# martingleich/RayTracingInAWeekend

Hardware: AMD Instinct MI355X
Metric: Msamples/sec at 1920x1080x512spp; achieved HBM GB/s vs peak (higher is better)
Workload: dtype f32

## Files before the change

include/rtw.h:

```cpp
#ifndef RTW_H
#define RTW_H

#include <stddef.h>
#include <stdint.h>

#ifdef __cplusplus
extern "C" {
#endif

#define RTW_API __attribute__((visibility("default")))
#define RTW_ABI_VERSION 2

#define RTW_OK 0
#define RTW_ERR_INVALID_ARGUMENT 1
#define RTW_ERR_NO_DEVICE 2
#define RTW_ERR_HIP 3
#define RTW_ERR_OUT_OF_MEMORY 4
#define RTW_ERR_UNSUPPORTED 5
#define RTW_ERR_IO 6
#define RTW_ERR_PARSE 7

#define RTW_GEOM_SPHERE 0
#define RTW_GEOM_RECT 1
#define RTW_GEOM_BOX 2
// ... 175 lines not shown
                                float* out_rgb, rtw_progress_fn cb, void* user);

RTW_API int rtw_render_devices(const rtw_world* world, const rtw_render_params* params, const int* devices,
                               int n_devices, float* out_rgb);
typedef struct rtw_multi rtw_multi;
RTW_API int rtw_multi_create(const rtw_world* world, const int* devices, int n_devices, rtw_multi** out);
RTW_API int rtw_multi_render(rtw_multi* m, const rtw_render_params* params, float* d_image);
RTW_API int rtw_multi_release(rtw_multi* m);
RTW_API int rtw_multi_peer_copies(const rtw_multi* m, uint64_t* copies);

RTW_API int rtw_world_upload(const rtw_world* world, int device, rtw_gpu_world** out);
RTW_API int rtw_world_release(rtw_gpu_world* gw);
RTW_API int rtw_world_tuning(rtw_gpu_world* gw, int* trace_min);
RTW_API int rtw_world_kernel(rtw_gpu_world* gw, int* lds_mode, int* leaf_kinds, int* tex_kinds, int* tree);
RTW_API int rtw_world_kernel_name(rtw_gpu_world* gw, char* buf, int cap);
RTW_API int rtw_world_last_frame(rtw_gpu_world* gw, int* launches, int* whole_pixel, int* trace_min);
RTW_API int rtw_world_last_frame_lists(rtw_gpu_world* gw, int* listed, int* empty, int* walked, double* mean_len);
RTW_API int rtw_world_primary_lists(rtw_gpu_world* gw, int32_t* n_tiles, int32_t* cap, double* build_ms,
                                    int32_t* count, int32_t* list);
RTW_API int rtw_primary_lists_host(const rtw_world* world, const rtw_render_params* params, int32_t cap,
                                   int32_t* count, int32_t* list);
RTW_API int rtw_render_device(rtw_gpu_world* gw, const rtw_render_params* params, float* d_out,
                              void* stream);
typedef struct rtw_accum rtw_accum;
#define RTW_ACCUM_MOMENTS 1u
#define RTW_ACCUM_ADAPTIVE 2u
#define RTW_ACCUM_FINITE 4u
typedef struct rtw_accum_info {
    uint32_t version;
    uint32_t flags;
// ... 187 lines not shown
```

raytracinginaweekend_amd/_native.py:

```python
from __future__ import annotations

import ctypes as C
import os

_HERE = os.path.dirname(os.path.abspath(__file__))
LIB_PATH = os.environ.get("RTW_LIBRARY") or os.path.join(_HERE, "librtw.so")

RTW_OK = 0
RTW_ERR_INVALID_ARGUMENT = 1
RTW_ERR_NO_DEVICE = 2
RTW_ERR_HIP = 3
RTW_ERR_OUT_OF_MEMORY = 4
RTW_ERR_UNSUPPORTED = 5
RTW_ERR_IO = 6
RTW_ERR_PARSE = 7

GEOM_SPHERE, GEOM_RECT, GEOM_BOX, GEOM_TRIANGLE = 0, 1, 2, 3
PLANE_XY, PLANE_XZ, PLANE_YZ = 0, 1, 2
MAT_LAMBERT, MAT_METAL, MAT_DIELECTRIC, MAT_DIFFUSE_LIGHT, MAT_ISOTROPIC = 0, 1, 2, 3, 4
TEX_SOLID, TEX_CHECKER, TEX_MARBLE, TEX_IMAGE = 0, 1, 2, 3
BG_SKY, BG_SOLID = 0, 1
MODE_DEFAULT, MODE_NORMALS = 0, 1
LEAF_VOLUME, LEAF_TRANSFORM, LEAF_ANIMATION = 1, 2, 4
LAYOUT_IMAGE, LAYOUT_TILES = 0, 1
# ... 254 lines not shown

ABI_VERSION = 2
_lib = None

_P = C.c_void_p
_SIGS = {
    "rtw_version": (C.c_int, []),
    "rtw_last_error": (C.c_char_p, []),
    "rtw_device_count": (C.c_int, [C.POINTER(C.c_int)]),
    "rtw_render": (C.c_int, [C.POINTER(World), C.POINTER(RenderParams), C.c_int, C.POINTER(C.c_float)]),
    "rtw_world_upload": (C.c_int, [C.POINTER(World), C.c_int, C.POINTER(_P)]),
    "rtw_world_release": (C.c_int, [_P]),
    "rtw_world_tuning": (C.c_int, [_P, C.POINTER(C.c_int)]),
    "rtw_world_kernel": (C.c_int, [_P] + [C.POINTER(C.c_int)] * 4),
    "rtw_world_kernel_name": (C.c_int, [_P, C.c_char_p, C.c_int]),
    "rtw_world_last_frame": (C.c_int, [_P] + [C.POINTER(C.c_int)] * 3),
    "rtw_world_last_frame_lists": (C.c_int, [_P] + [C.POINTER(C.c_int)] * 3 + [C.POINTER(C.c_double)]),
    "rtw_world_primary_lists": (C.c_int, [_P, C.POINTER(C.c_int32), C.POINTER(C.c_int32), C.POINTER(C.c_double),
                                          C.POINTER(C.c_int32), C.POINTER(C.c_int32)]),
    "rtw_primary_lists_host": (C.c_int, [C.POINTER(World), C.POINTER(RenderParams), C.c_int32, C.POINTER(C.c_int32),
                                         C.POINTER(C.c_int32)]),
    "rtw_render_device": (C.c_int, [_P, C.POINTER(RenderParams), _P, _P]),
    "rtw_render_devices": (C.c_int, [C.POINTER(World), C.POINTER(RenderParams), C.POINTER(C.c_int), C.c_int,
                                     C.POINTER(C.c_float)]),
    "rtw_multi_create": (C.c_int, [C.POINTER(World), C.POINTER(C.c_int), C.c_int, C.POINTER(_P)]),
    "rtw_multi_render": (C.c_int, [_P, C.POINTER(RenderParams), _P]),
    "rtw_multi_release": (C.c_int, [_P]),
    "rtw_multi_peer_copies": (C.c_int, [_P, C.POINTER(C.c_uint64)]),
    "rtw_world_fingerprint": (C.c_int, [C.POINTER(World), C.POINTER(C.c_uint64)]),
    "rtw_accum_create": (C.c_int, [_P, C.POINTER(RenderParams), C.c_uint32, C.POINTER(_P)]),
# ... 149 lines not shown
```

raytracinginaweekend_amd/csrc/rtw_device.hip:

```cpp
#include <hip/hip_runtime.h>

#include <algorithm>
#include <cmath>
#include <limits>
#include <cstdio>
#include <cstdlib>
#include <cstring>
#include <ctime>
#include <string>
#include <type_traits>
#include <vector>

#include "../../include/rtw_scalar.h"
#include "../../include/rtw_cull.h"
#include "../../include/rtw_beam.h"
#include "../../include/rtw_adapt.h"
#include "../../include/rtw_finite.h"
#include "../../include/rtw_parts.h"
#include "rtw_common.h"

#ifndef RTW_BLOCK
#define RTW_BLOCK 1024
#endif
#ifndef RTW_MIN_WAVES_PER_SIMD
// ... 143 lines not shown
    int32_t whole_pixel;
    const uint32_t* tile_perm;
    uint32_t* slot_cost;
    uint32_t chunks;
    uint64_t big_from;
    FastDiv fd_total, fd_rank, fd_tile, fd_tiles_x, fd_tile_w;
    FastDiv fd_spread, fd_epoch, fd_half;
    int32_t sh_xf, sh_sph, sh_bx, sh_rect;
    int32_t sphere_count, box_count;
    int32_t mb_off, mb_cap;
    int32_t tri_prefix, tri_stride;
    int32_t tri_prefix_mat, tri_prefix_w;
    const int32_t* pl_count;
    const int32_t* pl_list;
    int32_t pl_cap, pl_shade_min;
};

struct V3 {
    float x, y, z;
};
__host__ __device__ __forceinline__ V3 v3(float x, float y, float z) { return V3{x, y, z}; }
__host__ __device__ __forceinline__ V3 add(V3 a, V3 b) { return v3(a.x + b.x, a.y + b.y, a.z + b.z); }
__host__ __device__ __forceinline__ V3 sub(V3 a, V3 b) { return v3(a.x - b.x, a.y - b.y, a.z - b.z); }
__device__ __forceinline__ V3 neg(V3 a) { return v3(-a.x, -a.y, -a.z); }
__host__ __device__ __forceinline__ V3 mul(V3 a, float s) { return v3(a.x * s, a.y * s, a.z * s); }
__device__ __forceinline__ V3 divs(V3 a, float s) { return v3(a.x / s, a.y / s, a.z / s); }
__device__ __forceinline__ V3 conv(V3 a, V3 b) { return v3(a.x * b.x, a.y * b.y, a.z * b.z); }
__host__ __device__ __forceinline__ float dot(V3 a, V3 b) { return a.x * b.x + a.y * b.y + a.z * b.z; }
__host__ __device__ __forceinline__ V3 cross(V3 a, V3 b) {
    return v3(a.y * b.z - a.z * b.y, a.z * b.x - a.x * b.z, a.x * b.y - a.y * b.x);
// ... 946 lines not shown
        float d0, d1;
        d_unit_disc(&rng, d0, d1);
        off = mul(add(mul(ld3(c.unit_right), d0), mul(ld3(c.unit_up), d1)), c.lens_radius);
    }
    float start;
    if (c.time0 == c.time1) start = c.time0;
    else start = d_gen_range_f32(c.time0, c.time1, &rng);
    Ray r;
    r.time = start + (c.shutter_pace[0] * px + c.shutter_pace[1] * py);
    r.o = add(ld3(c.position), off);
    r.d = unit_x(sub(sub(add(ld3(c.upper_left_corner), mul(ld3(c.scaled_right), px)), mul(ld3(c.scaled_up), py)), off));
    return r;
}

#ifdef RTW_PHASE_TIMING
__device__ unsigned long long rtw_phase_cycles[8];
__device__ __forceinline__ unsigned long long* pt_slot() {
    __shared__ unsigned long long s[(RTW_BLOCK / 64) * 10];
    return s + (threadIdx.x >> 6) * 10;
}
#define RTW_PT_DECL do { unsigned long long* s_ = pt_slot(); if ((threadIdx.x & 63) == 0) { for (int k_ = 0; k_ < 8; ++k_) s_[k_] = 0; s_[8] = clock64(); s_[9] = 0; } } while (0);
#define RTW_PT(k) do { if ((int)(threadIdx.x & 63) == __ffsll((long long)__ballot(1)) - 1) { unsigned long long* s_ = pt_slot(); const unsigned long long now_ = clock64(); s_[s_[9]] += now_ - s_[8]; s_[8] = now_; s_[9] = (k); } } while (0)
#define RTW_PT_FLUSH do { RTW_PT(0); if ((threadIdx.x & 63) == 0) for (int k_ = 0; k_ < 8; ++k_) atomicAdd(&rtw_phase_cycles[k_], pt_slot()[k_]); } while (0)
#else
#define RTW_PT_DECL
#define RTW_PT(k) do { } while (0)
#define RTW_PT_FLUSH do { } while (0)
#endif

struct Path {
    Ray ray;
    V3 att, acc;
    int32_t depth;
    rtw_xoro rng;
};
struct ShadeOut {
    Path p;
    V3 color;
    int32_t done;
    uint32_t texels;
};
// ... 121 lines not shown
                }
        }
    } else {
        color = add(acc, conv(att, background(w.wc->bg, pdot)));
        done = true;
    }
    ShadeOut o;
    o.p = P;
    o.color = color;
    o.done = done ? 1 : 0;
    o.texels = STATS ? st.c[ST_TEXEL] : 0u;
    return o;
}

__device__ unsigned long long rtw_drain_counts[3];

#ifdef RTW_WAVE_TIMING
__device__ unsigned long long rtw_wave_times[3 * 8192];
__device__ unsigned long long rtw_wave_dry[8192];
__device__ unsigned long long rtw_wave_extra[8 * 8192];
#endif

enum { PH_PIXEL = 0, PH_TRACE = 1, PH_SHADE = 2, PH_REF = 3, PH_DONE = 4 };
enum { TM_REF = 0, TM_SAH = 1, TM_FALLBACK = 2 };
#define RTW_TF_SAH 16
#define RTW_TF_TIE 32


struct Trav {
    Ray ray;
// ... 348 lines not shown
        if (__builtin_amdgcn_readfirstlane((int)ok)) {
            j = (int)(si & 0xFFu);
            return uu;
        }
    }
}

__device__ __forceinline__ void sah_take(Trav& T, float t, int leaf) {
    const bool same = T.found >= 0 && t == __int_as_float(__float_as_int(T.te) - 1);
    const bool tie = same && T.found != leaf;
    T.fast = same ? (tie ? (T.fast | RTW_TF_TIE) : T.fast) : (T.fast & ~RTW_TF_TIE);
    T.te = same ? T.te : __int_as_float(__float_as_int(t) + 1);
    T.found = same ? T.found : leaf;
}

template <bool STATS, int LDS, int LK, int TX, bool GEN, bool WP, bool PL = false>
__device__ __forceinline__ void render_body(const KArgs& A) {
    static_assert(!PL || (LDS == 1 && LK == LK_SPHERES && !GEN), "leaf lists: plain-sphere worlds, LDS mode 1");
    constexpr bool LDS_SCENE = LDS >= 1;
    const DWorld& w = A.w;
    constexpr bool SAHK = LK <= LK_WRAPPED;
    const bool sah = SAHK && A.sah != 0;
    if (LDS_SCENE) {
        const float4* ga = sah ? w.sah_a : w.node_a;
        const float4* gb = sah ? w.sah_b : w.node_b;
        for (int i = threadIdx.x; i < A.node_count; i += RTW_BLOCK) {
            smem[i] = ga[i];
            smem[A.node_count + i] = gb[i];
        }
        const int32_t n_rec = A.leaf_count - A.tri_prefix;
        for (int i = threadIdx.x; i < n_rec; i += RTW_BLOCK) smem[2 * A.node_count + i] = w.leaf_fast[A.tri_prefix + i];
        const bool km_rec = sah && LK == LK_SPHERES;
        const int32_t km_f4 = km_rec ? 0 : (A.node_count + 1) / 2;
// ... 80 lines not shown
        fresh = true;
        if (PL) cam = true;
        RTW_PT(back);
    };

    int32_t trace_min = A.trace_min;
    bool tuned = true;
    if (A.tune) {
        const int ch = __hip_atomic_load(&A.tune->chosen, __ATOMIC_RELAXED, __HIP_MEMORY_SCOPE_AGENT);
        if (ch > 0) trace_min = ch;
        else tuned = A.tune_items == 0;
    }
    uint64_t w_next = 0, w_end = 0;
    uint32_t wq = (blockIdx.x * (RTW_BLOCK / 64) + (threadIdx.x >> 6)) % RTW_QUEUES;
    uint32_t qfail = 0;
    unsigned long long pf_b = 0;
    uint64_t pf_size = 0;
    int pf_lane = 0;
    auto prefetch = [&](int leader) {
        const uint64_t rest = A.q_cap > w_end ? A.q_cap - w_end : 0;
        const uint64_t cap = w_end * RTW_QUEUES >= A.big_from ? RTW_WAVE_BATCH_BIG : RTW_WAVE_BATCH;
        pf_size = max((uint64_t)1, min(cap, (uint64_t)fdiv((uint32_t)rest, A.fd_spread)));
        if (lane == leader) pf_b = atomicAdd(A.queue + wq * RTW_QSTRIDE, (unsigned long long)pf_size);
        pf_lane = leader;
    };
    RTW_PT_DECL
#ifdef RTW_WAVE_TIMING
    uint32_t wx_busy = 0, wx_n = 0, wx_sum = 0, wx_max = 0, wx_coop = 0, wx_ref = 0;
    uint64_t wx_tref = 0, wx_tsah = 0, wx_tcoop = 0;
    bool wx_dry = false;
#endif
    static_assert(!(GEN && WP), "GEN kernels take whole-pixel items at run time");
    const bool WPX = GEN ? A.whole_pixel != 0 : WP;
    constexpr bool SHARE_K = !STATS && LDS_SCENE && LK == LK_TRIS;
    int32_t mb_v = SHARE_K ? A.mb_off : -1;
    asm volatile("" : "+v"(mb_v));
    auto share_on = [&]() { return SHARE_K && __builtin_amdgcn_readfirstlane(mb_v) >= 0; };
    auto mailbox = [&]() { return reinterpret_cast<uint32_t*>(smem + __builtin_amdgcn_readfirstlane(mb_v)); };
    for (;;) {
        if (__ballot(T.phase != PH_DONE) == 0) break;
        RTW_PT(1);
        for (;;) {
            const unsigned long long m = __ballot(T.phase == PH_PIXEL);
            if (m == 0) break;
            if (qfail >= RTW_QUEUES) {
#ifdef RTW_WAVE_TIMING
                {
                    const uint32_t wv_ = (blockIdx.x * RTW_BLOCK + threadIdx.x) / 64;
                    if (wv_ < 8192) atomicMin(&rtw_wave_dry[wv_], (unsigned long long)wall_clock64());
                }
#endif
#ifdef RTW_WAVE_TIMING
                if (!wx_dry) wx_busy = (uint32_t)__popcll(__ballot(T.phase != PH_PIXEL));
                wx_dry = true;
#endif
                if (T.phase == PH_PIXEL) T.phase = PH_DONE;
// ... 13 lines not shown
                empty = base >= A.q_cap;
                w_next = empty ? A.q_cap : base;
                w_end = empty ? A.q_cap : min(base + size, A.q_cap);
                if (!tuned && wq == 0 && !empty) {
                    const uint64_t H = A.fd_half.d;
                    const uint64_t g0 = base * RTW_QUEUES, g1 = (base + size) * RTW_QUEUES;
                    const uint64_t j = fdiv((uint32_t)min(g0 + H - 1, (uint64_t)0xFFFFFFFFu), A.fd_half);
                    if (lane == leader && j >= 1 && j <= RTW_TUNE_STAMPS && j * H < g1)
                        __hip_atomic_store(&A.tune->tb[j - 1], wall_clock64(), __ATOMIC_RELAXED,
                                           __HIP_MEMORY_SCOPE_AGENT);
                }
            }
            const uint64_t left = min(need, w_end - w_next);
            const uint64_t first = w_next;
            w_next += left;
            if (!tuned) {
                const uint64_t e = fdiv((uint32_t)min(w_next * RTW_QUEUES, (uint64_t)0xFFFFFFFFu), A.fd_epoch);
                if (e == 0) {
                    trace_min = A.trace_min;
                } else if (e <= RTW_TUNE_EPOCHS) {
                    const int i = (int)e - 1;
                    trace_min = kTuneCand[i < RTW_TUNE_NCAND ? i : RTW_TUNE_EPOCHS - 1 - i];
                } else {
                    const unsigned long long* tbp = A.tune->tb;
                    auto stamp = [&](int k) {
                        return __hip_atomic_load(&tbp[k], __ATOMIC_RELAXED, __HIP_MEMORY_SCOPE_AGENT);
                    };
                    bool ok = stamp(0) != ~0ull && stamp(1) != ~0ull;
                    unsigned long long best_t = 0;
                    int best = A.trace_min;
// ... 66 lines not shown
                wq = (wq + 1) % RTW_QUEUES;
                ++qfail;
                w_next = w_end = 0;
            } else if (took) {
                qfail = 0;
            }
        }

        RTW_PT(2);
        uint64_t c_trav = 0;
        if (STATS) {
            c_trav = clock64();
            if (lane == __ffsll((long long)__ballot(1)) - 1)
                atomicAdd(&A.stats[ST_COUNT + DB_REST_CYCLES], (unsigned long long)(c_trav - c_mark));
        }
        if (fresh) {
            fresh = false;
            const RayPre rp = ray_pre(T.ray, A.mk_world != 0);
            T.inv = rp.inv;
            T.fast = (rp.fast ? 8 : 0) | (T.ray.d.x > 0.0f ? 1 : 0) | (T.ray.d.y > 0.0f ? 2 : 0) | (T.ray.d.z > 0.0f ? 4 : 0);
            T.node = w.root;
            if (sah) {
                if (rp.fast) {
                    T.node = LK == LK_SPHERES ? w.sah_root_c2 : w.sah_root;
                    T.fast |= RTW_TF_SAH;
                } else {
                    T.phase = PH_REF;
                }
            }
            T.sp = 0;
            T.te = F32_INF;
            T.found = -1;
            if (STATS) st.c[ST_RAYS]++;
            if constexpr (PL) {
                if (cam && rp.fast && sah) {
                    const uint32_t tile = (uint32_t)A.part_index + fdiv(slot, A.fd_tile) * (uint32_t)A.part_count;
                    const int32_t n = A.pl_count[tile];
                    if (n >= 0) {
                        const int32_t* __restrict__ L = A.pl_list + (size_t)tile * (uint32_t)A.pl_cap;
                        const float4* fast = smem + A.fast_off;
                        for (int32_t j = 0; j < n; ++j) {
                            const int32_t leaf = L[j];
                            float t;
                            if (STATS) st.c[ST_T_SPHERE]++;
                            if (sphere_t(fast[leaf], T.ray, 0.001f, T.te, t)) sah_take(T, t, leaf);
                        }
                        T.phase = PH_SHADE;
                    }
                }
            }
        }

        RTW_PT(3);
        if (sah) {
            const bool dry_coop = !STATS && LK <= LK_PLAIN && qfail >= RTW_QUEUES && A.coop_max > 0;
#ifdef RTW_WAVE_TIMING
            uint64_t wx_t0 = wall_clock64();
#endif
            int32_t tmin = __builtin_amdgcn_readfirstlane(trace_min);
            if (PL && (int32_t)__popcll(__ballot(T.phase == PH_SHADE)) >= A.pl_shade_min) tmin = 65;
            T = traverse<STATS, LDS, LK, true, TM_SAH>(A.wdev, stabs, T, tmin, A.node_count,
                                                       A.leaf_count, A.rect_count, A.tri_prefix, A.tri_stride, stack_off,
                                                       STATS ? A.stats + ST_COUNT : nullptr, dry_coop ? A.coop_max : -1);
// ... 185 lines not shown
                }
                if (STATS) st.c[ST_SAMPLES]++;
                const int32_t bounces = A.max_depth - depth;
                if (!STATS && A.slot_cost && bounces > 3) {
                    if (WPX) pcost += (uint32_t)bounces;
                    else atomicAdd(&A.slot_cost[slot], (uint32_t)bounces);
                }
#ifdef RTW_WAVE_TIMING
                if (qfail >= RTW_QUEUES) {
                    ++wx_n;
                    wx_sum += (uint32_t)bounces;
                    wx_max = max(wx_max, (uint32_t)bounces);
                }
#endif
                ++sample;
                if (sample >= sample_end) {
                    T.phase = PH_PIXEL;
                    if (WPX) {
                        if (!STATS && A.slot_cost && pcost) atomicAdd(&A.slot_cost[slot], pcost);
                        const V3 px = divs(psum, (float)A.spp);
                        float* o = A.layout == RTW_LAYOUT_TILES ? A.out + 3 * (size_t)slot : A.out + 3 * (size_t)pix;
                        o[0] = px.x;
                        o[1] = px.y;
                        o[2] = px.z;
                    }
                } else {
                    start_sample(7);
                }
            } else {
                fresh = true;
                if (PL) cam = false;
// ... 22 lines not shown
            a.sgn = __float_as_int(q1.w);
            a.inv = v3(q2.x, q2.y, q2.z);
            const CHit h = coop_solve<LDS, LK>(w, a, A.node_count, A.leaf_count, A.rect_count, A.fast_off, A.tri_prefix,
                                               A.tri_stride, A.coop_ties == 2);
            if (lane == 0) {
                mb_answer(mb, q, u, h);
                __hip_atomic_fetch_add(&mb[34], 1u, __ATOMIC_RELAXED, __HIP_MEMORY_SCOPE_WORKGROUP);
            }
        }
        __syncthreads();
        if (threadIdx.x < 3) {
            const uint32_t c = __hip_atomic_load(&mb[33 + threadIdx.x], __ATOMIC_RELAXED, __HIP_MEMORY_SCOPE_WORKGROUP);
            if (c) atomicAdd(&rtw_drain_counts[threadIdx.x], (unsigned long long)c);
        }
    }
    RTW_PT_FLUSH;
#ifdef RTW_WAVE_TIMING
    {
        const uint32_t wv_ = (blockIdx.x * RTW_BLOCK + threadIdx.x) / 64;
        if (wv_ < 8192) {
            unsigned long long* x = rtw_wave_extra + 8 * wv_;
            if (wx_busy) atomicMax(&x[0], (unsigned long long)wx_busy);
            atomicAdd(&x[1], (unsigned long long)wx_n);
            atomicAdd(&x[2], (unsigned long long)wx_sum);
            (void)wx_max;
            if (lane == 0) {
                x[4] = wx_coop;
                x[5] = wx_ref;
                x[6] = wx_tref;
                x[7] = wx_tsah;
// ... 15 lines not shown
#endif
    render_body<STATS, LDS, LK, TX, GEN, WP>(A);
#ifdef RTW_WAVE_TIMING
    const uint32_t wv = (blockIdx.x * RTW_BLOCK + threadIdx.x) / 64;
    if ((threadIdx.x & 63) == 0 && wv < 8192) {
        rtw_wave_times[3 * wv] = t_start;
        rtw_wave_times[3 * wv + 1] = wall_clock64();
        rtw_wave_times[3 * wv + 2] = rtw_wave_dry[wv];
        rtw_wave_dry[wv] = ~0ull;
    }
#endif
}
template <bool STATS, int LDS, int LK, int TX, bool GEN = false, bool WP = false>
__global__ __launch_bounds__(RTW_BLOCK, RTW_MIN_WAVES_PER_SIMD) void render_kernel_pl(KArgs A) {
    render_body<STATS, LDS, LK, TX, GEN, WP, true>(A);
}

#define RTW_PL_GROUP 64
__global__ __launch_bounds__(RTW_PL_GROUP) void primary_lists_kernel(const rtw_camera* __restrict__ cam,
                                                                      const float4* __restrict__ fast, int32_t leaf_count,
                                                                      int32_t W, int32_t H, int32_t tw, int32_t th,
                                                                      int32_t tiles_x, int32_t n_tiles, int32_t cap,
                                                                      int32_t* __restrict__ count, int32_t* __restrict__ list) {
    const int32_t tile = (int32_t)blockIdx.x;
    if (tile >= n_tiles) return;
    const int lane = threadIdx.x;
    rtw_beam_tile t;
    rtw_beam_tile_setup(cam, W, H, tw, th, tile % tiles_x, tile / tiles_x, &t);
    int32_t n = 0;
    bool walk = !t.ok;
// ... 1138 lines not shown
    uint64_t order_key[10] = {};
    hipEvent_t done = nullptr;
    bool done_recorded = false;
    uint32_t order_tiles = 0;
    bool order_valid = false;
    int32_t last_kernel[6] = {-1, -1, -1, -1, -1, -1};
    int32_t last_frame[4] = {-1, -1, -1, 0};
    bool pl_scope = false;
    int32_t* pl_buf = nullptr;
    int32_t pl_key[5] = {0, 0, 0, 0, 0};
    int32_t pl_tiles = 0;
    int32_t pl_info[3] = {0, 0, 0};
    double pl_mean = 0.0;
    double pl_build_ms = 0.0;
    int32_t last_pl = 0;
    int32_t last_lists[3] = {0, 0, 0};
    double last_mean = 0.0;
    uint64_t fingerprint = 0;
    std::vector<struct rtw_accum*> accums;
    std::vector<struct rtw_aov*> aovs;
};

extern "C" RTW_API int rtw_debug_wave_times(unsigned long long* out24576) {
#ifdef RTW_WAVE_TIMING
    HIP_TRY(hipDeviceSynchronize());
    HIP_TRY(hipMemcpyFromSymbol(out24576, HIP_SYMBOL(rtw_wave_times), 3 * 8192 * sizeof(unsigned long long)));
    return RTW_OK;
#else
    (void)out24576;
    return rtw::fail(RTW_ERR_UNSUPPORTED, "built without RTW_WAVE_TIMING");
// ... 12 lines not shown
#endif
}

extern "C" RTW_API int rtw_debug_drain_counts(int device, unsigned long long* out3, int reset) {
    if (!out3) return rtw::fail(RTW_ERR_INVALID_ARGUMENT, "null argument");
    HIP_TRY(hipSetDevice(device));
    HIP_TRY(hipDeviceSynchronize());
    HIP_TRY(hipMemcpyFromSymbol(out3, HIP_SYMBOL(rtw_drain_counts), 3 * sizeof(unsigned long long)));
    if (reset) {
        unsigned long long z[3] = {};
        HIP_TRY(hipMemcpyToSymbol(HIP_SYMBOL(rtw_drain_counts), z, sizeof(z)));
    }
    return RTW_OK;
}

extern "C" RTW_API int rtw_debug_phase_cycles(unsigned long long* out8) {
#ifdef RTW_PHASE_TIMING
    HIP_TRY(hipDeviceSynchronize());
    HIP_TRY(hipMemcpyFromSymbol(out8, HIP_SYMBOL(rtw_phase_cycles), 8 * sizeof(unsigned long long)));
    unsigned long long z[8] = {};
    HIP_TRY(hipMemcpyToSymbol(HIP_SYMBOL(rtw_phase_cycles), z, sizeof(z)));
    return RTW_OK;
#else
    (void)out8;
    return rtw::fail(RTW_ERR_UNSUPPORTED, "built without RTW_PHASE_TIMING");
#endif
}

extern "C" RTW_API int rtw_device_count(int* count) {
    if (!count) return rtw::fail(RTW_ERR_INVALID_ARGUMENT, "null count");
    int n = 0;
    hipError_t e = hipGetDeviceCount(&n);
    if (e != hipSuccess) n = 0;
    *count = n;
    return RTW_OK;
}

extern "C" RTW_API int rtw_world_upload(const rtw_world* w, int device, rtw_gpu_world** out) {
    if (!out) return rtw::fail(RTW_ERR_INVALID_ARGUMENT, "null out");
// ... 384 lines not shown
}

extern "C" RTW_API int rtw_world_kernel(rtw_gpu_world* g, int* lds_mode, int* leaf_kinds, int* tex_kinds, int* tree) {
    if (!g || !lds_mode || !leaf_kinds || !tex_kinds || !tree) return rtw::fail(RTW_ERR_INVALID_ARGUMENT, "null argument");
    *lds_mode = g->last_kernel[0];
    *leaf_kinds = g->last_kernel[1];
    *tex_kinds = g->last_kernel[2];
    *tree = g->last_kernel[3];
    return RTW_OK;
}

extern "C" RTW_API int rtw_world_kernel_name(rtw_gpu_world* g, char* buf, int cap) {
    if (!g || !buf || cap < 1) return rtw::fail(RTW_ERR_INVALID_ARGUMENT, "null argument");
    char s[64] = "";
    if (g->last_kernel[0] >= 0)
        std::snprintf(s, sizeof(s), "render_kernel%s<false, %d, %d, %d, %s, %s>", g->last_pl ? "_pl" : "", g->last_kernel[0], g->last_kernel[1],
                      g->last_kernel[2], g->last_kernel[4] ? "true" : "false", g->last_kernel[5] ? "true" : "false");
    if ((int)std::strlen(s) >= cap) return rtw::fail(RTW_ERR_INVALID_ARGUMENT, "buffer too small");
    std::memcpy(buf, s, std::strlen(s) + 1);
    return RTW_OK;
}

extern "C" RTW_API int rtw_world_last_frame(rtw_gpu_world* g, int* launches, int* whole_pixel, int* trace_min) {
    if (!g || !launches || !whole_pixel || !trace_min) return rtw::fail(RTW_ERR_INVALID_ARGUMENT, "null argument");
    *launches = g->last_frame[0];
    *whole_pixel = g->last_frame[1];
    *trace_min = g->last_frame[2];
    if (g->last_frame[3]) {
        HIP_TRY(hipSetDevice(g->device));
        int v = 0;
        HIP_TRY(hipMemcpy(&v, &g->tune->chosen, sizeof(int), hipMemcpyDeviceToHost));
        if (v > 0) *trace_min = v;
// ... 45 lines not shown
                                      w->leaf_count, cap, list + (size_t)t * cap);
    return RTW_OK;
}

static void accum_orphan(struct rtw_accum* a);
static void aov_orphan(struct rtw_aov* a);

extern "C" RTW_API int rtw_world_release(rtw_gpu_world* g) {
    if (!g) return RTW_OK;
    (void)hipSetDevice(g->device);
    for (struct rtw_accum* a : g->accums) accum_orphan(a);
    for (struct rtw_aov* a : g->aovs) aov_orphan(a);
    if (g->arena) (void)hipFree(g->arena);
    if (g->queue) (void)hipFree(g->queue);
    if (g->colors) (void)hipFree(g->colors);
    if (g->tune) (void)hipFree(g->tune);
    if (g->slot_cost) (void)hipFree(g->slot_cost);
    if (g->tile_buf) (void)hipFree(g->tile_buf);
    if (g->sort_tmp) (void)hipFree(g->sort_tmp);
    if (g->running) (void)hipFree(g->running);
    if (g->pl_buf) (void)hipFree(g->pl_buf);
    if (g->done) (void)hipEventDestroy(g->done);
    delete g;
    return RTW_OK;
}

namespace {

int make_args(const rtw_gpu_world* g, const rtw_render_params* p, KArgs& A) {
    if (!g || !p) return rtw::fail(RTW_ERR_INVALID_ARGUMENT, "null argument");
// ... 42 lines not shown
    A.wdev = g->wdev;
    A.trace_min = 32;
    A.stats_tree = 0;
    if (const char* e = getenv("RTW_TRACE_MIN")) A.trace_min = atoi(e);
    A.seed_key = rtw_seed_key(p->seed);
    A.sx = 1.0f / (float)(p->width - 1);
    A.sy = 1.0f / (float)(p->height - 1);
    A.ux = rtw_uniform_new(0.0f, 1.0f / (float)(p->width - 1));
    A.uy = rtw_uniform_new(0.0f, 1.0f / (float)(p->height - 1));
    return RTW_OK;
}

enum LaunchKind { LK_RENDER, LK_STATS };
size_t env_size(const char* name, size_t dflt);
constexpr int RTW_ACC_NO_WP = -1;
int launch_render(rtw_gpu_world* g, KArgs& A, int kind, hipStream_t stream, bool acc_wp = false) {
    const bool stats = kind == LK_STATS;
    const bool ktree = stats && A.stats_tree == 1;
    int lk = g->leaf_kinds, tx = g->tex_kinds;
    if (const char* e = std::getenv("RTW_LEAF_KINDS")) lk = std::max(lk, std::min(4, std::atoi(e)));
    if (const char* e = std::getenv("RTW_TEX_KINDS")) tx = std::max(tx, std::min(1, std::atoi(e)));
    const bool sah = (!stats || ktree) && g->sah_nodes > 0 && g->mk_world && lk <= LK_WRAPPED &&
                     g->sah_folded == (lk == LK_SPHERES);
    A.sah = sah ? 1 : 0;
    A.coop_max = g->leaf_count <= RTW_COOP_LEAVES ? (int32_t)env_size("RTW_COOP_MAX", RTW_COOP_MAX) : 0;
    if (const char* e = std::getenv("RTW_COOP_MAX"))
        if (e[0] == '0') A.coop_max = 0;
    A.coop_ties = g->leaf_count <= RTW_COOP_LEAVES && g->w.leaf_key != nullptr ? 1 : 0;
    if (const char* e = std::getenv("RTW_COOP_TIES"))
        if (e[0] == '0') A.coop_ties = 0;
    if (const char* e = std::getenv("RTW_COOP_AUDIT"))
        if (e[0] == '1' && A.coop_ties) A.coop_ties = 2;
    const int blocks_per_cu = std::max(1, (4 * RTW_MIN_WAVES_PER_SIMD * 64) / RTW_BLOCK);
    size_t cap = std::min({(size_t)RTW_LDS_SCENE_MAX, (size_t)g->lds_max, (size_t)g->lds_cu / blocks_per_cu});
#ifdef RTW_PHASE_TIMING
    cap -= (RTW_BLOCK / 64) * 10 * sizeof(unsigned long long);
#endif
    const size_t stack_bytes = (size_t)g->depth * RTW_BLOCK * sizeof(int32_t);
    const size_t stack16_bytes = stack_bytes / 2;
    const char* lds_mode_env = std::getenv("RTW_LDS_MODE");
    A.node_count = sah ? g->sah_nodes : g->node_count;
    const int kernel_lk = stats && !sah ? (int)LK_ANY : lk;
    A.tri_prefix = kernel_lk == LK_TRIS ? g->tri_prefix : 0;
    A.tri_stride = kernel_lk == LK_TRIS ? std::max(1, g->tri_count) : RTW_TRI_SOA;
    const size_t tri_bytes = (size_t)4 * A.tri_stride * sizeof(float4);
    const size_t scene_bytes =
        (size_t)(2 * A.node_count + g->leaf_count - A.tri_prefix + (sah && lk == LK_SPHERES ? 0 : (A.node_count + 1) / 2) +
                 2 * g->rect_count) * sizeof(float4);
    A.fast_off = 2 * A.node_count - A.tri_prefix;
    if (A.fast_off < 0) return rtw::fail(RTW_ERR_UNSUPPORTED, "triangle prefix longer than the node records");
    int mode = 0;
// ... 75 lines not shown
#undef RTW_SSET
#define RTW_GSET(TX)                                                                                     \
    {{render_kernel<false, 1, LK_WRAPPED, TX, true>, render_kernel<false, 2, LK_WRAPPED, TX, true>}, \
     {render_kernel<false, 1, LK_ANY, TX, true>, render_kernel<false, 2, LK_ANY, TX, true>}}
    static const KFn fns_gen[2][2][2] = {RTW_GSET(TX_SOLID), RTW_GSET(TX_ANY)};
#undef RTW_GSET
    const bool gen = !stats && A.sh_xf >= 0;
    if (gen && tx != TX_SOLID && A.sh_tex0 >= 0)
        return rtw::fail(RTW_ERR_UNSUPPORTED, "GEN kernel with a texture table in LDS");
    if (gen && acc_wp) return RTW_ACC_NO_WP;
    const int wp = A.whole_pixel ? 1 : 0;
    KFn kf = stats ? (sah ? fns_stats_sah[lk][mode] : fns_stats[mode])
             : gen   ? fns_gen[tx][lk - LK_WRAPPED][mode - 1]
                     : fns[wp][tx][lk][mode];
    static const KFn fns_pl[2][2] = {
        {render_kernel_pl<false, 1, LK_SPHERES, TX_SOLID, false, false>, render_kernel_pl<false, 1, LK_SPHERES, TX_ANY, false, false>},
        {render_kernel_pl<false, 1, LK_SPHERES, TX_SOLID, false, true>, render_kernel_pl<false, 1, LK_SPHERES, TX_ANY, false, true>}};
    const bool pl = (!stats || ktree) && !gen && A.pl_count != nullptr && sah && lk == LK_SPHERES && mode == 1;
    if (pl) kf = stats ? render_kernel_pl<true, 1, LK_SPHERES, TX_ANY> : fns_pl[wp][tx];
    else A.pl_count = nullptr;
    if (!stats) {
        g->last_pl = pl ? 1 : 0;
        g->last_kernel[0] = mode;
        g->last_kernel[1] = lk;
        g->last_kernel[2] = tx;
        g->last_kernel[3] = sah ? 1 : 0;
        g->last_kernel[4] = gen ? 1 : 0;
        g->last_kernel[5] = gen ? 0 : wp;
    }
    const void* fn = (const void*)kf;
    HIP_TRY(hipFuncSetAttribute(fn, hipFuncAttributeMaxDynamicSharedMemorySize, (int)lds));
    int per_cu = 0;
    HIP_TRY(hipOccupancyMaxActiveBlocksPerMultiprocessor(&per_cu, fn, RTW_BLOCK, lds));
    if (per_cu < 1) return rtw::fail(RTW_ERR_UNSUPPORTED, "render kernel does not fit on a CU");
    const int64_t want = (int64_t)((A.items + RTW_BLOCK - 1) / RTW_BLOCK);
    const int64_t blocks = std::max<int64_t>(1, std::min<int64_t>(want, (int64_t)per_cu * g->cus));
    HIP_TRY(hipMemsetAsync(A.queue, 0, RTW_QUEUE_BLOCK * sizeof(unsigned long long), stream));
    A.tune_items = 0;
    if (A.tune && A.total > 0 && !A.tile_perm) {
        const uint64_t lanes = (uint64_t)blocks * RTW_BLOCK;
        const uint64_t E = (uint64_t)A.total * ((2 * lanes + A.total - 1) / A.total);
        if (A.items_big >= (uint64_t)(RTW_TUNE_EPOCHS + 2) * E) {
            A.tune_items = E;
            HIP_TRY(hipMemsetAsync(A.tune->tb, 0xFF, sizeof(A.tune->tb), stream));
        }
    }
    A.fd_spread = fastdiv_make((uint32_t)std::max<int64_t>(1, RTW_BATCH_SPREAD * blocks * (RTW_BLOCK / 64) / RTW_QUEUES));
    A.fd_epoch = fastdiv_make((uint32_t)std::max<uint64_t>(1, A.tune_items));
    A.fd_half = fastdiv_make((uint32_t)std::max<uint64_t>(1, A.tune_items / 2));
    hipLaunchKernelGGL(kf, dim3((unsigned)blocks), dim3(RTW_BLOCK), lds, stream, A);
    HIP_TRY(hipGetLastError());
// ... 1383 lines not shown
```

raytracinginaweekend_amd/rendering.py:

```python
from __future__ import annotations

import ctypes as C
import enum
from dataclasses import dataclass

import numpy as np

from . import _native as N
from ._native import check, lib
from .world import World


class RenderMode(enum.IntEnum):
    Default = N.MODE_DEFAULT
    Normals = N.MODE_NORMALS


@dataclass(frozen=True)
class Size2i:
    width: int
    height: int

    def count(self) -> int:
        return self.width * self.height
# ... 131 lines not shown
        v = C.c_int()
        check(lib().rtw_world_tuning(self._h, C.byref(v)))
        return v.value

    def kernel_variant(self) -> dict:
        m, lk, tx, tr = C.c_int(), C.c_int(), C.c_int(), C.c_int()
        check(lib().rtw_world_kernel(self._h, C.byref(m), C.byref(lk), C.byref(tx), C.byref(tr)))
        name = C.create_string_buffer(64)
        check(lib().rtw_world_kernel_name(self._h, name, 64))
        out = {"lds_mode": m.value, "leaf_kinds": lk.value, "tex_kinds": tx.value,
               "tree": ("reference", "sah")[tr.value] if tr.value >= 0 else None,
               "name": name.value.decode()}
        out.update(self._lists())
        return out

    def last_frame(self) -> dict:
        if not hasattr(lib(), "rtw_world_last_frame"):
            return {"launches": None, "whole_pixel": None, "trace_min": self.tuned_trace_min()}
        n, wp, tm = C.c_int(), C.c_int(), C.c_int()
        check(lib().rtw_world_last_frame(self._h, C.byref(n), C.byref(wp), C.byref(tm)))
        out = {"launches": n.value, "whole_pixel": bool(wp.value == 1), "trace_min": tm.value}
        out.update(self._lists())
        return out

    def _lists(self) -> dict:
        if not hasattr(lib(), "rtw_world_last_frame_lists"):
            return {}
        a, b, c, m = C.c_int(), C.c_int(), C.c_int(), C.c_double()
        check(lib().rtw_world_last_frame_lists(self._h, C.byref(a), C.byref(b), C.byref(c), C.byref(m)))
        return {"tiles_listed": a.value, "tiles_empty": b.value, "tiles_walked": c.value,
# ... 55 lines not shown
```

Measured before the change: 8771.

## Batch camera-ray generation per wave and park rays in a global buffer

```diff
diff --git a/include/rtw.h b/include/rtw.h
--- a/include/rtw.h
+++ b/include/rtw.h
@@ -213,6 +213,7 @@
 RTW_API int rtw_world_tuning(rtw_gpu_world* gw, int* trace_min);
 RTW_API int rtw_world_kernel(rtw_gpu_world* gw, int* lds_mode, int* leaf_kinds, int* tex_kinds, int* tree);
 RTW_API int rtw_world_kernel_name(rtw_gpu_world* gw, char* buf, int cap);
+RTW_API int rtw_debug_park_counts(int device, unsigned long long* out3, int reset);
 RTW_API int rtw_world_last_frame(rtw_gpu_world* gw, int* launches, int* whole_pixel, int* trace_min);
 RTW_API int rtw_world_last_frame_lists(rtw_gpu_world* gw, int* listed, int* empty, int* walked, double* mean_len);
 RTW_API int rtw_world_primary_lists(rtw_gpu_world* gw, int32_t* n_tiles, int32_t* cap, double* build_ms,
diff --git a/raytracinginaweekend_amd/_native.py b/raytracinginaweekend_amd/_native.py
--- a/raytracinginaweekend_amd/_native.py
+++ b/raytracinginaweekend_amd/_native.py
@@ -292,6 +292,7 @@
     "rtw_world_tuning": (C.c_int, [_P, C.POINTER(C.c_int)]),
     "rtw_world_kernel": (C.c_int, [_P] + [C.POINTER(C.c_int)] * 4),
     "rtw_world_kernel_name": (C.c_int, [_P, C.c_char_p, C.c_int]),
+    "rtw_debug_park_counts": (C.c_int, [C.c_int, C.POINTER(C.c_ulonglong), C.c_int]),
     "rtw_world_last_frame": (C.c_int, [_P] + [C.POINTER(C.c_int)] * 3),
     "rtw_world_last_frame_lists": (C.c_int, [_P] + [C.POINTER(C.c_int)] * 3 + [C.POINTER(C.c_double)]),
     "rtw_world_primary_lists": (C.c_int, [_P, C.POINTER(C.c_int32), C.POINTER(C.c_int32), C.POINTER(C.c_double),
diff --git a/raytracinginaweekend_amd/csrc/rtw_device.hip b/raytracinginaweekend_amd/csrc/rtw_device.hip
--- a/raytracinginaweekend_amd/csrc/rtw_device.hip
+++ b/raytracinginaweekend_amd/csrc/rtw_device.hip
@@ -181,6 +181,7 @@
     const int32_t* pl_count;
     const int32_t* pl_list;
     int32_t pl_cap, pl_shade_min;
+    float4* park;
 };
 
 struct V3 {
@@ -1157,17 +1158,20 @@
 }
 
 #ifdef RTW_PHASE_TIMING
-__device__ unsigned long long rtw_phase_cycles[8];
+#define RTW_PT_SUMS 12
+__device__ unsigned long long rtw_phase_cycles[RTW_PT_SUMS];
 __device__ __forceinline__ unsigned long long* pt_slot() {
-    __shared__ unsigned long long s[(RTW_BLOCK / 64) * 10];
-    return s + (threadIdx.x >> 6) * 10;
-}
-#define RTW_PT_DECL do { unsigned long long* s_ = pt_slot(); if ((threadIdx.x & 63) == 0) { for (int k_ = 0; k_ < 8; ++k_) s_[k_] = 0; s_[8] = clock64(); s_[9] = 0; } } while (0);
-#define RTW_PT(k) do { if ((int)(threadIdx.x & 63) == __ffsll((long long)__ballot(1)) - 1) { unsigned long long* s_ = pt_slot(); const unsigned long long now_ = clock64(); s_[s_[9]] += now_ - s_[8]; s_[8] = now_; s_[9] = (k); } } while (0)
-#define RTW_PT_FLUSH do { RTW_PT(0); if ((threadIdx.x & 63) == 0) for (int k_ = 0; k_ < 8; ++k_) atomicAdd(&rtw_phase_cycles[k_], pt_slot()[k_]); } while (0)
+    __shared__ unsigned long long s[(RTW_BLOCK / 64) * (RTW_PT_SUMS + 2)];
+    return s + (threadIdx.x >> 6) * (RTW_PT_SUMS + 2);
+}
+#define RTW_PT_DECL do { unsigned long long* s_ = pt_slot(); if ((threadIdx.x & 63) == 0) { for (int k_ = 0; k_ < RTW_PT_SUMS; ++k_) s_[k_] = 0; s_[RTW_PT_SUMS] = clock64(); s_[RTW_PT_SUMS + 1] = 0; } } while (0);
+#define RTW_PT(k) do { if ((int)(threadIdx.x & 63) == __ffsll((long long)__ballot(1)) - 1) { unsigned long long* s_ = pt_slot(); const unsigned long long now_ = clock64(); s_[s_[RTW_PT_SUMS + 1]] += now_ - s_[RTW_PT_SUMS]; s_[RTW_PT_SUMS] = now_; s_[RTW_PT_SUMS + 1] = (k); } } while (0)
+#define RTW_PT_ROUND(leader, lanes) do { if ((int)(threadIdx.x & 63) == (leader)) { unsigned long long* s_ = pt_slot(); s_[10] += 1; s_[11] += (lanes); } } while (0)
+#define RTW_PT_FLUSH do { RTW_PT(0); if ((threadIdx.x & 63) == 0) for (int k_ = 0; k_ < RTW_PT_SUMS; ++k_) atomicAdd(&rtw_phase_cycles[k_], pt_slot()[k_]); } while (0)
 #else
 #define RTW_PT_DECL
 #define RTW_PT(k) do { } while (0)
+#define RTW_PT_ROUND(leader, lanes) do { } while (0)
 #define RTW_PT_FLUSH do { } while (0)
 #endif
 
@@ -1319,6 +1323,8 @@
 }
 
 __device__ unsigned long long rtw_drain_counts[3];
+__device__ unsigned long long rtw_park_counts[3];
+#define RTW_PARK_GROUPS 5
 
 #ifdef RTW_WAVE_TIMING
 __device__ unsigned long long rtw_wave_times[3 * 8192];
@@ -1697,9 +1703,10 @@
     T.found = same ? T.found : leaf;
 }
 
-template <bool STATS, int LDS, int LK, int TX, bool GEN, bool WP, bool PL = false>
+template <bool STATS, int LDS, int LK, int TX, bool GEN, bool WP, bool PL = false, bool CB = false>
 __device__ __forceinline__ void render_body(const KArgs& A) {
     static_assert(!PL || (LDS == 1 && LK == LK_SPHERES && !GEN), "leaf lists: plain-sphere worlds, LDS mode 1");
+    static_assert(!CB || (PL && !WP && !STATS), "camera batch: the leaf-list kernel's single-sample variants");
     constexpr bool LDS_SCENE = LDS >= 1;
     const DWorld& w = A.w;
     constexpr bool SAHK = LK <= LK_WRAPPED;
@@ -1810,6 +1817,8 @@
     uint64_t w_next = 0, w_end = 0;
     uint32_t wq = (blockIdx.x * (RTW_BLOCK / 64) + (threadIdx.x >> 6)) % RTW_QUEUES;
     uint32_t qfail = 0;
+    uint32_t p_next = 0, p_count = 0;
+    uint32_t pk_fills = 0, pk_stored = 0, pk_picked = 0;
     unsigned long long pf_b = 0;
     uint64_t pf_size = 0;
     int pf_lane = 0;
@@ -1836,6 +1845,170 @@
     for (;;) {
         if (__ballot(T.phase != PH_DONE) == 0) break;
         RTW_PT(1);
+        if constexpr (CB) {
+            for (;;) {
+                const unsigned long long m = __ballot(T.phase == PH_PIXEL);
+                if (m == 0) break;
+                if (p_next == p_count) {
+                    if (qfail >= RTW_QUEUES) {
+#ifdef RTW_WAVE_TIMING
+                        {
+                            const uint32_t wv_ = (blockIdx.x * RTW_BLOCK + threadIdx.x) / 64;
+                            if (wv_ < 8192) atomicMin(&rtw_wave_dry[wv_], (unsigned long long)wall_clock64());
+                        }
+                        if (!wx_dry) wx_busy = (uint32_t)__popcll(__ballot(T.phase != PH_PIXEL));
+                        wx_dry = true;
+#endif
+                        if (T.phase == PH_PIXEL) T.phase = PH_DONE;
+                        continue;
+                    }
+                    const int leader = __ffsll((long long)m) - 1;
+                    bool empty = false, took = false;
+                    if (w_next == w_end) {
+                        if (pf_size == 0) prefetch(leader);
+                        const uint64_t base =
+                            ((uint64_t)(uint32_t)__builtin_amdgcn_readlane((int)(uint32_t)(pf_b >> 32), pf_lane) << 32) |
+                            (uint64_t)(uint32_t)__builtin_amdgcn_readlane((int)(uint32_t)pf_b, pf_lane);
+                        const uint64_t size = pf_size;
+                        pf_size = 0;
+                        took = true;
+                        empty = base >= A.q_cap;
+                        w_next = empty ? A.q_cap : base;
+                        w_end = empty ? A.q_cap : min(base + size, A.q_cap);
+                    }
+                    const uint32_t left = (uint32_t)min((uint64_t)64, w_end - w_next);
+                    const uint64_t first = w_next;
+                    w_next += left;
+                    if (left) RTW_PT_ROUND(leader, (uint64_t)__popcll(m));
+                    bool valid = false;
+                    if ((uint32_t)lane < left) {
+                        const uint64_t loc = first + (uint32_t)lane;
+                        const uint64_t item = ((loc / RTW_QGRAN) * RTW_QUEUES + wq) * RTW_QGRAN + loc % RTW_QGRAN;
+                        uint32_t f_slot = 0, f_sample = 0;
+                        int32_t f_px = 0, f_py = 0;
+                        if (item < A.items) {
+                            const bool big = item < A.items_big;
+                            const uint32_t rel = (uint32_t)(big ? item : item - A.items_big);
+                            uint32_t ck, c, lt, it;
+                            if (A.tile_perm) {
+                                const uint32_t g = fdiv(rel, A.fd_rank);
+                                const uint32_t wi = rel - g * A.fd_rank.d;
+                                ck = fdiv(wi, A.fd_tile);
+                                it = wi - ck * A.fd_tile.d;
+                                lt = A.tile_perm[g];
+                                c = lt * A.fd_tile.d + it;
+                            } else {
+                                ck = fdiv(rel, A.fd_total);
+                                c = rel - ck * A.total;
+                                lt = fdiv(c, A.fd_tile);
+                                it = c - lt * A.fd_tile.d;
+                            }
+                            const uint32_t tile = (uint32_t)A.part_index + lt * (uint32_t)A.part_count;
+                            const uint32_t ty = fdiv(tile, A.fd_tiles_x), iy = fdiv(it, A.fd_tile_w);
+                            f_px = (int32_t)((tile - ty * (uint32_t)A.tiles_x) * (uint32_t)A.tile_w + (it - iy * (uint32_t)A.tile_w));
+                            f_py = (int32_t)(ty * (uint32_t)A.tile_h + iy);
+                            valid = f_px < A.width && f_py < A.height;
+                            f_slot = c;
+                            f_sample = big ? A.s_begin + ck * A.chunk : A.s_split + ck;
+                        }
+                        float4* P = A.park + ((size_t)(blockIdx.x * (RTW_BLOCK / 64) + (threadIdx.x >> 6)) * RTW_PARK_GROUPS) * 64 + lane;
+                        if (valid) {
+                            RTW_PT(5);
+                            const uint32_t f_pix = (uint32_t)(f_py * A.width + f_px);
+                            rtw_xoro f_rng = rtw_sample_stream(A.seed_key, f_pix, f_sample);
+                            const float jx = d_uniform_sample(A.ux, &f_rng);
+                            const float jy = d_uniform_sample(A.uy, &f_rng);
+                            Trav F;
+                            F.ray = camera_ray(w.wc->cam, f_rng, (float)f_px * A.sx + jx, (float)f_py * A.sy + jy);
+                            RTW_PT(8);
+                            const RayPre rp = ray_pre(F.ray, A.mk_world != 0);
+                            F.fast = (rp.fast ? 8 : 0) | (F.ray.d.x > 0.0f ? 1 : 0) | (F.ray.d.y > 0.0f ? 2 : 0) | (F.ray.d.z > 0.0f ? 4 : 0);
+                            F.phase = PH_TRACE;
+                            F.te = F32_INF;
+                            F.found = -1;
+                            if (sah) {
+                                if (rp.fast) F.fast |= RTW_TF_SAH;
+                                else F.phase = PH_REF;
+                            }
+                            if (rp.fast && sah) {
+                                const uint32_t tile = (uint32_t)A.part_index + fdiv(f_slot, A.fd_tile) * (uint32_t)A.part_count;
+                                const int32_t n = A.pl_count[tile];
+                                if (n >= 0) {
+                                    const int32_t* __restrict__ L = A.pl_list + (size_t)tile * (uint32_t)A.pl_cap;
+                                    const float4* fast = smem + A.fast_off;
+                                    for (int32_t j = 0; j < n; ++j) {
+                                        const int32_t leaf = L[j];
+                                        float t;
+                                        if (sphere_t(fast[leaf], F.ray, 0.001f, F.te, t)) sah_take(F, t, leaf);
+                                    }
+                                    F.phase = PH_SHADE;
+                                }
+                            }
+                            RTW_PT(1);
+                            P[0 * 64] = make_float4(F.ray.o.x, F.ray.o.y, F.ray.o.z, F.ray.time);
+                            P[1 * 64] = make_float4(F.ray.d.x, F.ray.d.y, F.ray.d.z, F.te);
+                            P[2 * 64] = make_float4(rp.inv.x, rp.inv.y, rp.inv.z, __int_as_float(F.fast | (F.phase << 8) | (1 << 16)));
+                            P[3 * 64] = make_float4(__int_as_float((int)(uint32_t)f_rng.s0), __int_as_float((int)(uint32_t)(f_rng.s0 >> 32)),
+                                                    __int_as_float((int)(uint32_t)f_rng.s1), __int_as_float((int)(uint32_t)(f_rng.s1 >> 32)));
+                            P[4 * 64] = make_float4(__int_as_float(F.found), __int_as_float((int)f_slot), __int_as_float((int)f_sample), 0.0f);
+                        } else {
+                            P[2 * 64] = make_float4(0.0f, 0.0f, 0.0f, 0.0f);
+                        }
+                    }
+                    if (left) {
+                        ++pk_fills;
+                        pk_stored += (uint32_t)__popcll(__ballot(valid));
+                        p_next = 0;
+                        p_count = left;
+                        __builtin_amdgcn_fence(__ATOMIC_RELEASE, "wavefront");
+                        __builtin_amdgcn_fence(__ATOMIC_ACQUIRE, "wavefront");
+                    }
+                    if (empty) {
+                        wq = (wq + 1) % RTW_QUEUES;
+                        ++qfail;
+                        w_next = w_end = 0;
+                    } else if (took) {
+                        qfail = 0;
+                    }
+                    if (!left) continue;
+                }
+                const uint32_t avail = p_count - p_next;
+                bool got = false;
+                if (T.phase == PH_PIXEL) {
+                    const unsigned long long below = (lane == 0) ? 0ull : (m & (~0ull >> (64 - lane)));
+                    const uint32_t r = (uint32_t)__popcll(below);
+                    if (r < avail) {
+                        const float4* P = A.park + ((size_t)(blockIdx.x * (RTW_BLOCK / 64) + (threadIdx.x >> 6)) * RTW_PARK_GROUPS) * 64 + (p_next + r);
+                        const float4 q2 = P[2 * 64];
+                        const int32_t bits = __float_as_int(q2.w);
+                        if (bits >> 16) {
+                            const float4 q0 = P[0 * 64], q1 = P[1 * 64], q3 = P[3 * 64], q4 = P[4 * 64];
+                            T.ray.o = v3(q0.x, q0.y, q0.z);
+                            T.ray.time = q0.w;
+                            T.ray.d = v3(q1.x, q1.y, q1.z);
+                            T.te = q1.w;
+                            T.inv = v3(q2.x, q2.y, q2.z);
+                            T.fast = bits & 0xFF;
+                            T.phase = (bits >> 8) & 0xFF;
+                            T.rng.s0 = (uint64_t)(uint32_t)__float_as_int(q3.x) | ((uint64_t)(uint32_t)__float_as_int(q3.y) << 32);
+                            T.rng.s1 = (uint64_t)(uint32_t)__float_as_int(q3.z) | ((uint64_t)(uint32_t)__float_as_int(q3.w) << 32);
+                            T.found = __float_as_int(q4.x);
+                            slot = (uint32_t)__float_as_int(q4.y);
+                            sample = (uint32_t)__float_as_int(q4.z);
+                            T.node = (T.fast & RTW_TF_SAH) ? w.sah_root_c2 : w.root;
+                            T.sp = 0;
+                            pdot = dot(v3(0.0f, 1.0f, 0.0f), T.ray.d);
+                            att = v3(1.0f, 1.0f, 1.0f);
+                            acc = v3(0.0f, 0.0f, 0.0f);
+                            depth = A.max_depth;
+                            got = true;
+                        }
+                    }
+                }
+                pk_picked += (uint32_t)__popcll(__ballot(got));
+                p_next += min((uint32_t)__popcll(m), avail);
+            }
+        } else
         for (;;) {
             const unsigned long long m = __ballot(T.phase == PH_PIXEL);
             if (m == 0) break;
@@ -1879,6 +2052,7 @@
             const uint64_t left = min(need, w_end - w_next);
             const uint64_t first = w_next;
             w_next += left;
+            if (left) RTW_PT_ROUND(leader, need);
             if (!tuned) {
                 const uint64_t e = fdiv((uint32_t)min(w_next * RTW_QUEUES, (uint64_t)0xFFFFFFFFu), A.fd_epoch);
                 if (e == 0) {
@@ -1975,6 +2149,9 @@
             if (lane == __ffsll((long long)__ballot(1)) - 1)
                 atomicAdd(&A.stats[ST_COUNT + DB_REST_CYCLES], (unsigned long long)(c_trav - c_mark));
         }
+#ifdef RTW_PHASE_TIMING
+        if (PL && __ballot(fresh && !cam) == 0 && __ballot(fresh) != 0) RTW_PT(8);
+#endif
         if (fresh) {
             fresh = false;
             const RayPre rp = ray_pre(T.ray, A.mk_world != 0);
@@ -1993,8 +2170,9 @@
             T.te = F32_INF;
             T.found = -1;
             if (STATS) st.c[ST_RAYS]++;
-            if constexpr (PL) {
+            if constexpr (PL && !CB) {
                 if (cam && rp.fast && sah) {
+                    RTW_PT(8);
                     const uint32_t tile = (uint32_t)A.part_index + fdiv(slot, A.fd_tile) * (uint32_t)A.part_count;
                     const int32_t n = A.pl_count[tile];
                     if (n >= 0) {
@@ -2008,6 +2186,7 @@
                         }
                         T.phase = PH_SHADE;
                     }
+                    RTW_PT(2);
                 }
             }
         }
@@ -2223,7 +2402,7 @@
                 }
 #endif
                 ++sample;
-                if (sample >= sample_end) {
+                if (CB || sample >= sample_end) {
                     T.phase = PH_PIXEL;
                     if (WPX) {
                         if (!STATS && A.slot_cost && pcost) atomicAdd(&A.slot_cost[slot], pcost);
@@ -2276,6 +2455,9 @@
             if (c) atomicAdd(&rtw_drain_counts[threadIdx.x], (unsigned long long)c);
         }
     }
+    if constexpr (CB) {
+        if (lane < 3) atomicAdd(&rtw_park_counts[lane], (unsigned long long)(lane == 0 ? pk_fills : lane == 1 ? pk_stored : pk_picked));
+    }
     RTW_PT_FLUSH;
 #ifdef RTW_WAVE_TIMING
     {
@@ -2321,6 +2503,11 @@
 template <bool STATS, int LDS, int LK, int TX, bool GEN = false, bool WP = false>
 __global__ __launch_bounds__(RTW_BLOCK, RTW_MIN_WAVES_PER_SIMD) void render_kernel_pl(KArgs A) {
     render_body<STATS, LDS, LK, TX, GEN, WP, true>(A);
+}
+template <bool STATS, int LDS, int LK, int TX, bool GEN, bool WP, bool CB>
+__global__ __launch_bounds__(RTW_BLOCK, RTW_MIN_WAVES_PER_SIMD) void render_kernel_pl(KArgs A) {
+    static_assert(!STATS && !WP, "seven places: the single-sample product kernels");
+    render_body<STATS, LDS, LK, TX, GEN, WP, true, CB>(A);
 }
 
 #define RTW_PL_GROUP 64
@@ -3489,6 +3676,9 @@
     double pl_mean = 0.0;
     double pl_build_ms = 0.0;
     int32_t last_pl = 0;
+    int32_t last_cb = 0;
+    float4* park = nullptr;
+    size_t park_bytes = 0;
     int32_t last_lists[3] = {0, 0, 0};
     double last_mean = 0.0;
     uint64_t fingerprint = 0;
@@ -3531,6 +3721,18 @@
     return RTW_OK;
 }
 
+extern "C" RTW_API int rtw_debug_park_counts(int device, unsigned long long* out3, int reset) {
+    if (!out3) return rtw::fail(RTW_ERR_INVALID_ARGUMENT, "null argument");
+    HIP_TRY(hipSetDevice(device));
+    HIP_TRY(hipDeviceSynchronize());
+    HIP_TRY(hipMemcpyFromSymbol(out3, HIP_SYMBOL(rtw_park_counts), 3 * sizeof(unsigned long long)));
+    if (reset) {
+        unsigned long long z[3] = {};
+        HIP_TRY(hipMemcpyToSymbol(HIP_SYMBOL(rtw_park_counts), z, sizeof(z)));
+    }
+    return RTW_OK;
+}
+
 extern "C" RTW_API int rtw_debug_phase_cycles(unsigned long long* out8) {
 #ifdef RTW_PHASE_TIMING
     HIP_TRY(hipDeviceSynchronize());
@@ -3540,6 +3742,20 @@
     return RTW_OK;
 #else
     (void)out8;
+    return rtw::fail(RTW_ERR_UNSUPPORTED, "built without RTW_PHASE_TIMING");
+#endif
+}
+
+extern "C" RTW_API int rtw_debug_phase_extra(unsigned long long* out4) {
+#ifdef RTW_PHASE_TIMING
+    HIP_TRY(hipDeviceSynchronize());
+    HIP_TRY(hipMemcpyFromSymbol(out4, HIP_SYMBOL(rtw_phase_cycles), 4 * sizeof(unsigned long long),
+                                8 * sizeof(unsigned long long)));
+    unsigned long long z[4] = {};
+    HIP_TRY(hipMemcpyToSymbol(HIP_SYMBOL(rtw_phase_cycles), z, sizeof(z), 8 * sizeof(unsigned long long)));
+    return RTW_OK;
+#else
+    (void)out4;
     return rtw::fail(RTW_ERR_UNSUPPORTED, "built without RTW_PHASE_TIMING");
 #endif
 }
@@ -3954,8 +4170,9 @@
     if (!g || !buf || cap < 1) return rtw::fail(RTW_ERR_INVALID_ARGUMENT, "null argument");
     char s[64] = "";
     if (g->last_kernel[0] >= 0)
-        std::snprintf(s, sizeof(s), "render_kernel%s<false, %d, %d, %d, %s, %s>", g->last_pl ? "_pl" : "", g->last_kernel[0], g->last_kernel[1],
-                      g->last_kernel[2], g->last_kernel[4] ? "true" : "false", g->last_kernel[5] ? "true" : "false");
+        std::snprintf(s, sizeof(s), "render_kernel%s<false, %d, %d, %d, %s, %s%s>", g->last_pl ? "_pl" : "", g->last_kernel[0], g->last_kernel[1],
+                      g->last_kernel[2], g->last_kernel[4] ? "true" : "false", g->last_kernel[5] ? "true" : "false",
+                      !g->last_pl || g->last_kernel[5] ? "" : g->last_cb ? ", true" : ", false");
     if ((int)std::strlen(s) >= cap) return rtw::fail(RTW_ERR_INVALID_ARGUMENT, "buffer too small");
     std::memcpy(buf, s, std::strlen(s) + 1);
     return RTW_OK;
@@ -4031,6 +4248,7 @@
     if (g->arena) (void)hipFree(g->arena);
     if (g->queue) (void)hipFree(g->queue);
     if (g->colors) (void)hipFree(g->colors);
+    if (g->park) (void)hipFree(g->park);
     if (g->tune) (void)hipFree(g->tune);
     if (g->slot_cost) (void)hipFree(g->slot_cost);
     if (g->tile_buf) (void)hipFree(g->tile_buf);
@@ -4103,6 +4321,7 @@
 enum LaunchKind { LK_RENDER, LK_STATS };
 size_t env_size(const char* name, size_t dflt);
 constexpr int RTW_ACC_NO_WP = -1;
+int grow(void** buf, size_t* have, size_t need);
 int launch_render(rtw_gpu_world* g, KArgs& A, int kind, hipStream_t stream, bool acc_wp = false) {
     const bool stats = kind == LK_STATS;
     const bool ktree = stats && A.stats_tree == 1;
@@ -4123,7 +4342,7 @@
     const int blocks_per_cu = std::max(1, (4 * RTW_MIN_WAVES_PER_SIMD * 64) / RTW_BLOCK);
     size_t cap = std::min({(size_t)RTW_LDS_SCENE_MAX, (size_t)g->lds_max, (size_t)g->lds_cu / blocks_per_cu});
 #ifdef RTW_PHASE_TIMING
-    cap -= (RTW_BLOCK / 64) * 10 * sizeof(unsigned long long);
+    cap -= (RTW_BLOCK / 64) * (RTW_PT_SUMS + 2) * sizeof(unsigned long long);
 #endif
     const size_t stack_bytes = (size_t)g->depth * RTW_BLOCK * sizeof(int32_t);
     const size_t stack16_bytes = stack_bytes / 2;
@@ -4229,12 +4448,19 @@
              : gen   ? fns_gen[tx][lk - LK_WRAPPED][mode - 1]
                      : fns[wp][tx][lk][mode];
     static const KFn fns_pl[2][2] = {
-        {render_kernel_pl<false, 1, LK_SPHERES, TX_SOLID, false, false>, render_kernel_pl<false, 1, LK_SPHERES, TX_ANY, false, false>},
+        {render_kernel_pl<false, 1, LK_SPHERES, TX_SOLID, false, false, false>, render_kernel_pl<false, 1, LK_SPHERES, TX_ANY, false, false, false>},
         {render_kernel_pl<false, 1, LK_SPHERES, TX_SOLID, false, true>, render_kernel_pl<false, 1, LK_SPHERES, TX_ANY, false, true>}};
     const bool pl = (!stats || ktree) && !gen && A.pl_count != nullptr && sah && lk == LK_SPHERES && mode == 1;
     if (pl) kf = stats ? render_kernel_pl<true, 1, LK_SPHERES, TX_ANY> : fns_pl[wp][tx];
     else A.pl_count = nullptr;
+    static const KFn fns_cb[2] = {render_kernel_pl<false, 1, LK_SPHERES, TX_SOLID, false, false, true>,
+                                  render_kernel_pl<false, 1, LK_SPHERES, TX_ANY, false, false, true>};
+    const char* cbe = std::getenv("RTW_CAMERA_BATCH");
+    const bool cb = pl && !stats && !wp && A.tune == nullptr && A.chunk == 1 && !(cbe && cbe[0] == '0');
+    if (cb) kf = fns_cb[tx];
+    A.park = nullptr;
     if (!stats) {
+        g->last_cb = cb ? 1 : 0;
         g->last_pl = pl ? 1 : 0;
         g->last_kernel[0] = mode;
         g->last_kernel[1] = lk;
@@ -4250,6 +4476,12 @@
     if (per_cu < 1) return rtw::fail(RTW_ERR_UNSUPPORTED, "render kernel does not fit on a CU");
     const int64_t want = (int64_t)((A.items + RTW_BLOCK - 1) / RTW_BLOCK);
     const int64_t blocks = std::max<int64_t>(1, std::min<int64_t>(want, (int64_t)per_cu * g->cus));
+    if (cb) {
+        const int rc = grow((void**)&g->park, &g->park_bytes,
+                            (size_t)blocks * (RTW_BLOCK / 64) * RTW_PARK_GROUPS * 64 * sizeof(float4));
+        if (rc != RTW_OK) return rc;
+        A.park = g->park;
+    }
     HIP_TRY(hipMemsetAsync(A.queue, 0, RTW_QUEUE_BLOCK * sizeof(unsigned long long), stream));
     A.tune_items = 0;
     if (A.tune && A.total > 0 && !A.tile_perm) {
diff --git a/raytracinginaweekend_amd/rendering.py b/raytracinginaweekend_amd/rendering.py
--- a/raytracinginaweekend_amd/rendering.py
+++ b/raytracinginaweekend_amd/rendering.py
@@ -169,6 +169,11 @@
         out.update(self._lists())
         return out
 
+    def park_counts(self, reset: bool = True) -> tuple:
+        buf = (C.c_ulonglong * 3)()
+        check(lib().rtw_debug_park_counts(self.device, buf, 1 if reset else 0))
+        return tuple(int(v) for v in buf)
+
     def last_frame(self) -> dict:
         if not hasattr(lib(), "rtw_world_last_frame"):
             return {"launches": None, "whole_pixel": None, "trace_min": self.tuned_trace_min()}
```

Measured after the change: 9006 (median of 6 runs). 1.03x the previous value.
